# kensho-technologies/pyctcdecode

Hardware: NVIDIA H100
Metric: logit frames/sec decoded (batch, beam=100) (higher is better)
Workload: dtype f64

## Files before the change

include/b200ctc.h:

```cpp
#ifndef B200CTC_H
#define B200CTC_H

#include <stddef.h>
#include <stdint.h>

#ifdef __cplusplus
extern "C" {
#endif

#define B2C_E_OK 0
#define B2C_E_ARG (-1)
#define B2C_E_CUDA (-2)
#define B2C_E_IO (-3)
#define B2C_E_NOMEM (-4)
#define B2C_E_INTERNAL (-5)

#define B2C_DTYPE_F32 0
#define B2C_DTYPE_F64 1
#define B2C_DTYPE_F16 2
#define B2C_DTYPE_BF16 3

typedef struct b2c_lm b2c_lm_t;
typedef struct b2c_decoder b2c_decoder_t;
typedef struct b2c_result b2c_result_t;
// ... 98 lines not shown
    const int32_t* n_stream_toks;
    const uint32_t* stream_toks;
    int64_t n_stream_toks_total;
    const char* stream_pieces;
    size_t stream_pieces_size;
    const int32_t* stream_boundary;
} b2c_packed_t;
int b2c_result_packed(b2c_result_t* res, b2c_packed_t* out);
#define B2C_KIND_CONT 0
#define B2C_KIND_SPACE 1
#define B2C_KIND_BPE 2
int b2c_result_stream_beam(const b2c_result_t* res, int utt, int beam, int32_t aux[4], const uint32_t** toks, int* n_toks);
int b2c_result_n_frames(const b2c_result_t* res, int utt, int beam);
int b2c_hash_utf8(const char* s, uint64_t* hash, uint32_t* n_chars);
int b2c_hash_utf8_batch(const char* data, size_t size, int64_t count, uint64_t* hashes, uint32_t* n_chars);
int b2c_decoder_token_id(const b2c_decoder_t* dec, const char* label);

typedef struct {
    float ms_prepare;
    float ms_beam;
    float ms_total;
    int launches;
    long long h2d_bytes, d2h_bytes;
    long long frames;
    long long tokens;
    int cap_candidates;
    int cta_threads;
    int cta_slots;
    long long oversize_frames;
    int kernel_variant;
    long long cand_hist[7];
    long long inplace_frames;
    long long sorted_frames;
    int hinted;
} b2c_timings_t;
int b2c_decoder_last_timings(const b2c_decoder_t* dec, b2c_timings_t* out);
int b2c_decoder_last_tokens(const b2c_decoder_t* dec, int64_t* n_frames, int64_t* n_entries, int32_t* counts, uint32_t* ids,
                            double* lps, uint16_t* rec_id0, double* rec_lp0, int32_t* is_prob);

#ifdef __cplusplus
}
#endif
#endif
```

pyctcdecode_b200/_lib.py:

```python
import ctypes as C
import os
import threading

_HERE = os.path.dirname(os.path.abspath(__file__))
DEFAULT_LIBRARY = os.path.join(_HERE, "libb200ctc.so")

_lock = threading.Lock()
_lib = None
_lib_path = None


class LMState(C.Structure):
    _fields_ = [("words", C.c_uint32 * 5), ("backoff", C.c_float * 5), ("length", C.c_uint32)]


class StreamBeam(C.Structure):
    _fields_ = [("part_hash", C.c_uint64), ("logit_score", C.c_double), ("word_off", C.c_uint32), ("n_words", C.c_uint32),
                ("part_len", C.c_uint32), ("last_tok", C.c_uint32), ("pf_s", C.c_int32), ("pf_e", C.c_int32)]


class StreamState(C.Structure):
    _fields_ = [("beams", C.POINTER(StreamBeam)), ("n_beams", C.c_int), ("processed_frames", C.c_int),
                ("word_hashes", C.POINTER(C.c_uint64)), ("word_lens", C.POINTER(C.c_uint32)), ("n_words", C.c_int)]

# ... 15 lines not shown
        ("stream_states", C.POINTER(StreamState)),
        ("finalize_mode", C.c_int),
        ("text_only", C.c_int),
    ]


class Packed(C.Structure):
    _fields_ = [("n_utts", C.c_int32), ("n_models", C.c_int32), ("n_beams_total", C.c_int64), ("n_words_total", C.c_int64),
                ("n_beams", C.POINTER(C.c_int32)), ("scores", C.POINTER(C.c_double)), ("n_words", C.POINTER(C.c_int32)),
                ("frames", C.POINTER(C.c_int32)), ("texts", C.c_void_p), ("texts_size", C.c_size_t),
                ("states", C.POINTER(LMState)), ("stream_aux", C.POINTER(C.c_int32)), ("n_stream_toks", C.POINTER(C.c_int32)),
                ("stream_toks", C.POINTER(C.c_uint32)), ("n_stream_toks_total", C.c_int64),
                ("stream_pieces", C.c_void_p), ("stream_pieces_size", C.c_size_t), ("stream_boundary", C.POINTER(C.c_int32))]


class Timings(C.Structure):
    _fields_ = [
        ("ms_prepare", C.c_float),
        ("ms_beam", C.c_float),
        ("ms_total", C.c_float),
        ("launches", C.c_int),
        ("h2d_bytes", C.c_longlong),
        ("d2h_bytes", C.c_longlong),
        ("frames", C.c_longlong),
        ("tokens", C.c_longlong),
        ("cap_candidates", C.c_int),
        ("cta_threads", C.c_int),
        ("cta_slots", C.c_int),
        ("oversize_frames", C.c_longlong),
        ("kernel_variant", C.c_int),
        ("cand_hist", C.c_longlong * 7),
        ("inplace_frames", C.c_longlong),
        ("sorted_frames", C.c_longlong),
        ("hinted", C.c_int),
    ]


def _declare(L):
    vp, cp, i32, f64 = C.c_void_p, C.c_char_p, C.c_int, C.c_double
    pp = C.POINTER(vp)
    L.b2c_last_error.restype = cp
    L.b2c_version.restype = i32
    L.b2c_device_count.restype = i32
    L.b2c_lm_build_from_arpa.argtypes = [cp, C.POINTER(cp), C.c_long, pp]
    L.b2c_lm_build_from_file.argtypes = [cp, C.POINTER(cp), C.c_long, pp]
    L.b2c_lm_blob.argtypes = [vp, pp, C.POINTER(C.c_size_t)]
    L.b2c_lm_from_blob.argtypes = [vp, C.c_size_t, pp]
    L.b2c_lm_upload.argtypes = [vp, i32]
    L.b2c_lm_adopt_device_blob.argtypes = [vp, i32, vp, C.c_size_t]
    L.b2c_lm_destroy.argtypes = [vp]
    L.b2c_lm_destroy.restype = None
    L.b2c_lm_order.argtypes = [vp]
    L.b2c_lm_contains.argtypes = [vp, cp]
    L.b2c_lm_in_unigrams.argtypes = [vp, cp]
    L.b2c_lm_has_prefix.argtypes = [vp, cp]
    L.b2c_lm_have_unigrams.argtypes = [vp]
    L.b2c_lm_begin_sentence.argtypes = [vp, C.POINTER(LMState)]
    L.b2c_lm_begin_sentence.restype = None
    L.b2c_lm_null_context.argtypes = [vp, C.POINTER(LMState)]
    L.b2c_lm_null_context.restype = None
    L.b2c_lm_base_score.argtypes = [vp, C.POINTER(LMState), cp, C.POINTER(LMState)]
    L.b2c_lm_base_score.restype = C.c_float
    L.b2c_decoder_create.argtypes = [C.POINTER(cp), i32, i32, vp, i32, pp]
    L.b2c_decoder_destroy.argtypes = [vp]
    L.b2c_decoder_destroy.restype = None
    L.b2c_decoder_set_params.argtypes = [vp, f64, f64, f64, i32]
# ... 85 lines not shown
```

pyctcdecode_b200/csrc/b2c_api.cu:

```cuda
#include <algorithm>
#include <chrono>
#include <cmath>
#include <cstdint>
#include <cstdlib>
#include <cstring>
#include <map>
#include <memory>
#include <mutex>
#include <numeric>
#include <string>
#include <thread>
#include <atomic>
#include <condition_variable>
#include <functional>
#include <vector>

#ifdef B2C_HOSTSIM
#include "cuda_shim.h"
#else
#include <cuda_runtime.h>
#endif

#include "../../include/b200ctc.h"
#include "b2c_beam.h"
// ... 607 lines not shown
    for (size_t i = 0; i < br.words.size(); ++i) {
        if (i) br.text += ' ';
        br.text += br.words[i];
    }
    br.frames.resize(static_cast<size_t>(nw) * 2);
    for (int w = 0; w < nw; ++w) {
        br.frames[2 * w] = frames[2 * (nw - 1 - w)];
        br.frames[2 * w + 1] = frames[2 * (nw - 1 - w) + 1];
    }
    const size_t n = std::min(br.words.size(), static_cast<size_t>(nw));
    br.words.resize(n);
    br.frames.resize(n * 2);
}

static const int kNumCaps = 6;
static const u32 kCaps[kNumCaps] = {128, 256, 512, 1024, 2048, 4096};
static int threads_of(int c) { return kCaps[c] <= 128 ? 32 : (kCaps[c] <= 256 ? 64 : (kCaps[c] >= 2048 ? 256 : 128)); }
static int per_sm_of(u32 smem_bytes, int threads) {
    const int by_smem = static_cast<int>(std::max<u64>(1, (224 * 1024) / std::max<u32>(smem_bytes + 1024, 2048)));
    return std::min(by_smem, threads == 32 ? 8 : (threads == 64 ? 4 : (threads >= 256 ? 1 : 2)));
}

struct Launch { int cls; size_t ord_off; int count; B2cLayout L; int slots; int per_sm; int threads; int v5; };
struct Geometry {
    int n_utts = 0, V = 0, beam_width = 0, W_tab = 0, n_lm = 1, s_max_beams = 0, T_max = 0;
    u64 s_max_words = 0, total_frames = 0;
    size_t esz = 4;
    bool streaming = false, hint_ok = false, pipelined = false;
    u32 smem_budget = 0;
    const int32_t* T = nullptr;
    const int* order = nullptr;
};
struct Knobs {
    bool host_prof, no_pipe, no_hinted, force_v5, no_v5, no_lean, force_lean, pipe_all, no_gate, gate_early;
    int v5_variant, force_chunks;
};
static bool env_set(const char* name) { return std::getenv(name) != nullptr; }
static Knobs read_knobs() {
    Knobs k;
    k.host_prof = env_set("B200CTC_HOST_PROFILE");
    k.no_pipe = env_set("B200CTC_NO_PIPELINE") || !env_switch("B200CTC_PIPELINE", B2C_DEFAULT_PIPELINE != 0);
    k.no_hinted = env_set("B200CTC_NO_HINTED");
    k.force_v5 = env_set("B200CTC_FORCE_V5");
    k.no_v5 = env_set("B200CTC_NO_V5");
    const char* v = std::getenv("B200CTC_V5_VARIANT"), *fc = std::getenv("B200CTC_FORCE_CHUNKS");
    k.v5_variant = v ? std::max(0, std::min(2, std::atoi(v))) : -1;
    k.no_lean = env_set("B200CTC_NO_LEAN") || !env_switch("B200CTC_LEAN", B2C_DEFAULT_LEAN != 0);
    k.force_lean = env_set("B200CTC_FORCE_LEAN");
    k.force_chunks = fc ? std::atoi(fc) : 0;
    k.pipe_all = env_set("B200CTC_PIPELINE_ALL"); k.no_gate = env_set("B200CTC_NO_GATE");
    k.gate_early = env_set("B200CTC_HOSTSIM_GATE_EARLY");
    return k;
}
struct Plan {
    std::vector<Launch> launches;
    std::vector<int> ord;
    bool use_v5 = false, use_lean = false;
    int v5_variant = 0;
    std::vector<int> bounds;
    bool gated = false;
    bool redo_plain = false;
};

struct MetaLayout {
    size_t T, run, ord, next, ptr, bytes;
    explicit MetaLayout(int n = 0)
        : T(al16(8ull * n)), run(T + al16(4ull * n)), ord(run + al16(8ull * (n + 1))), next(ord + 2 * al16(4ull * n)), ptr(next + 64),
          bytes(ptr + al16(8ull * n)) {}
};
struct OutViews {
    int *nbeams, *status; double* scores; int *ntok, *nwords; B2cLmState* states;
    int* aux;
    B2cLmState* states_x;
};
struct OutLayout {
    u64 st = 0, sc = 0, nt = 0, nw = 0, ls = 0, ax = 0, lx = 0, bytes = 0;
    bool has_aux = false, has_x = false;
    OutLayout() = default;
    OutLayout(int n, int OB, int n_lm, bool streaming)
        : st(al16(4ull * n)), sc(st + al16(4ull * n)), nt(sc + al16(16ull * OB * n)), nw(nt + al16(4ull * OB * n)), ls(nw + al16(4ull * OB * n)),
          ax(ls + al16(sizeof(B2cLmState) * static_cast<u64>(OB) * n)), lx(ax + (streaming ? al16(16ull * OB * n) : 0)),
          bytes(lx + al16(sizeof(B2cLmState) * static_cast<u64>(OB) * n * static_cast<u64>(n_lm - 1))), has_aux(streaming), has_x(n_lm > 1) {}
    OutViews at(u8* b) const {
        return OutViews{reinterpret_cast<int*>(b), reinterpret_cast<int*>(b + st), reinterpret_cast<double*>(b + sc),
// ... 633 lines not shown
            const b2c_stream_state_t& ss = o->stream_states[i];
            if (ss.n_beams < 0 || ss.n_beams > 65535 || (ss.n_beams > 0 && !ss.beams)) return fail(B2C_E_ARG, "bad stream state");
            const B2cStreamUtt su{static_cast<u32>(c.s_beams.size()), static_cast<u32>(ss.n_beams), ss.processed_frames, 0};
            const u32 wbase = static_cast<u32>(c.s_wh.size());
            u64 words = 0;
            for (int b = 0; b < ss.n_beams; ++b) {
                const b2c_stream_beam_t& ib = ss.beams[b];
                if (static_cast<u64>(ib.word_off) + ib.n_words > static_cast<u64>(std::max(ss.n_words, 0)))
                    return fail(B2C_E_ARG, "stream beam word range outside the state's word list");
                if (ib.last_tok != B2C_NO_TOK && ib.last_tok >= static_cast<u32>(g.V)) return fail(B2C_E_ARG, "stream beam last_tok out of range");
                const u32 last = ib.last_tok == B2C_NO_TOK ? B2C_NO_TOK : d->toks[ib.last_tok].canon;
                c.s_beams.push_back(B2cStreamBeam{ib.part_hash, ib.logit_score, wbase + ib.word_off, ib.n_words, ib.part_len, last, ib.pf_s, ib.pf_e});
                words += ib.n_words;
            }
            for (int w = 0; w < ss.n_words; ++w) { c.s_wh.push_back(ss.word_hashes[w]); c.s_wl.push_back(ss.word_lens[w]); }
            c.s_utts[i] = su;
            g.s_max_beams = std::max(g.s_max_beams, ss.n_beams);
            g.s_max_words = std::max(g.s_max_words, words);
        }
    }
    g.W_tab = std::max(o->beam_width, g.s_max_beams);
    return 0;
}

static int make_params(b2c_decoder* d, Call& c) {
    const b2c_decode_opts_t* o = c.opts;
    B2cParams& P = c.P;
    P.V = c.g.V; P.is_bpe = d->is_bpe; P.has_dup_labels = d->has_dup_labels;
    P.beam_width = o->beam_width; P.prune_history = o->prune_history ? 1 : 0; P.out_beams = c.OB; P.narrow_chain = c.text_only ? 1 : 0;
    P.prune_logp = o->beam_prune_logp; P.token_min_logp = o->token_min_logp;
    P.alpha = d->alpha; P.beta = d->beta; P.unk_offset = d->unk;
    P.log_base_change = 0x1.26bb1bbb55516p+1;
    P.score_boundary = d->score_boundary; P.hot_weight = o->hotword_weight; P.bucket_scale = b2c_bucket_scale(o->beam_prune_logp);
    P.toks = d->d_toks.as<B2cTok>();
    if (d->lm) {
        auto it = d->lm->dev.find(d->device);
        if (it == d->lm->dev.end()) return fail(B2C_E_INTERNAL, "language model is not resident on this device");
        P.lm = d->lm->host.view(it->second);
        if (P.lm.order > B2C_MAX_ORDER) return fail(B2C_E_ARG, "n-gram order too large");
        P.n_lm = 1 + static_cast<int>(d->lmx.size());
    }
    int max_order = P.lm.order;
    std::vector<B2cLmExtra> lmx_host(d->lmx.size());
    for (size_t j = 0; j < d->lmx.size(); ++j) {
        const b2c_decoder::ExtraLm& x = d->lmx[j];
        auto it = x.lm->dev.find(d->device);
        if (it == x.lm->dev.end()) return fail(B2C_E_INTERNAL, "language model is not resident on this device");
        B2cLmExtra& X = lmx_host[j];
        std::memset(&X, 0, sizeof(X));
        X.lm = x.lm->host.view(it->second);
        if (X.lm.order > B2C_MAX_ORDER) return fail(B2C_E_ARG, "n-gram order too large");
        X.alpha = x.alpha; X.beta = x.beta; X.unk_offset = x.unk; X.score_boundary = x.score_boundary;
        max_order = std::max(max_order, X.lm.order);
    }
    if (!lmx_host.empty()) {
        if (d->d_lmx.ensure(sizeof(B2cLmExtra) * lmx_host.size())) return B2C_E_NOMEM;
        CUDA_OK(cudaMemcpy(d->d_lmx.p, lmx_host.data(), sizeof(B2cLmExtra) * lmx_host.size(), cudaMemcpyHostToDevice));
        P.lmx = d->d_lmx.as<B2cLmExtra>();
    }
    c.g.n_lm = std::max(1, P.n_lm);
    P.hist_n = std::max(1, max_order - 1);
    build_hot(o, c.hot, P.n_hot, P.hot_min_len_all);
    if (d->d_hot.ensure(c.hot.size() * sizeof(B2cHot))) return B2C_E_NOMEM;
    P.hot = d->d_hot.as<B2cHot>(); P.hot_mask = c.hot.size() - 1;
    return 0;
}
// ... 315 lines not shown
    return 0;
}

static int read_outputs(b2c_decoder* d, const Call& c, bool frames) {
    CUDA_OK(cudaMemcpyAsync(d->h_out_small.p, d->d_out_small.p, c.out.bytes, cudaMemcpyDeviceToHost, d->stream));
    CUDA_OK(cudaMemcpyAsync(d->h_out_toks.p, d->d_out_toks.p, c.tok_bytes, cudaMemcpyDeviceToHost, d->stream));
    if (frames) CUDA_OK(cudaMemcpyAsync(d->h_out_frames.p, d->d_out_frames.p, c.frm_bytes, cudaMemcpyDeviceToHost, d->stream));
    return 0;
}

static int read_back(b2c_decoder* d, Call& c) {
    const int n = c.g.n_utts;
    cudaStream_t st = d->stream;
    B2C_TRY(read_outputs(d, c, !c.text_only));
    if (d->h_mstats.ensure(64)) return B2C_E_NOMEM;
    CUDA_OK(cudaMemcpyAsync(d->h_mstats.p, d->d_mstats.p, 64, cudaMemcpyDeviceToHost, st));
    if (c.g.pipelined) CUDA_OK(cudaMemcpyAsync(d->h_sumk.p, d->d_sumk.p, 4ull * n, cudaMemcpyDeviceToHost, st));
    CUDA_OK(cudaEventRecord(d->ev[4], st));
    c.hp.mark(2);
    CUDA_OK(cudaStreamSynchronize(st));
    c.hp.mark(3);
    if (c.g.pipelined && d->h_maxk.as<u32>()[0] != 0) return B2C_E_RETRY_PLAIN;
    if (c.gated_call) {
        const int* status = c.out.at(d->h_out_small.as<u8>()).status;
        for (int i = 0; i < n; ++i) if (status[i] & B2C_ERR_GATE) { d->pipe_refused = true; return B2C_E_RETRY_PLAIN; }
    }
    d->tm.d2h_bytes += static_cast<long long>(c.out.bytes + c.tok_bytes + (c.text_only ? 0 : c.frm_bytes) + 8ull * n + 32);
    const u32* ms = d->h_mstats.as<u32>();
    d->hint_valid = true;
    d->hint_beam = c.opts->beam_width; d->hint_lm = c.P.lm.order > 0 ? 1 : 0; d->hint_hot = c.P.n_hot > 0 ? 1 : 0; d->hint_prune = c.P.prune_history;
    for (int q = 0; q < 6; ++q) d->hint_over[q] = ms[q];
    d->hint_frames = ms[6];
    for (int q = 0; q < 7; ++q) d->tm.cand_hist[q] = ms[q];
    d->tm.inplace_frames = ms[7]; d->tm.sorted_frames = ms[8];
    d->hint_wide_utts = ms[9]; d->hint_utts = ms[10];
    d->tm.oversize_frames = 0;
    for (int q = 0; q < 6; ++q)
        if (static_cast<int>(128u << q) == d->tm.cap_candidates) d->tm.oversize_frames = ms[q];
    return 0;
}

static int retry_failed(b2c_decoder* d, Call& c) {
    const int n = c.g.n_utts;
    cudaStream_t st = d->stream;
    const int* status = c.out.at(d->h_out_small.as<u8>()).status;
    std::vector<int> failed;
    for (int i = 0; i < n; ++i) if (status[i] != B2C_OK) failed.push_back(i);
    if (c.plan.use_lean && 10 * failed.size() > static_cast<size_t>(n)) d->lean_bad = true;
    for (int pass = 0; pass < 2 && !failed.empty(); ++pass) {
        bool only_slots = c.plan.use_lean && pass == 0;
        for (int i : failed) only_slots = only_slots && status[i] == B2C_ERR_SLOTS;
        if (pass == 0 && !only_slots) continue;
        int cls = kNumCaps;
        if (only_slots) {
            c.plan.use_lean = false;
            cls = 0;
            for (const Launch& l0 : c.plan.launches) if (l0.v5 >= 0) cls = l0.cls;
        }
        const Launch ln = plan_launch(c.g, c.maxk, c.plan, d->n_sm, failed, cls, !only_slots, static_cast<size_t>(n));
        if (ln.L.smem_bytes > d->smem_optin) return fail(B2C_E_ARG, "beam_width too large for the shared-memory selection arrays");
        if (d->d_ws.ensure(static_cast<u64>(ln.slots) * ln.L.gws_bytes)) return B2C_E_NOMEM;
        int* h_ord = c.h_ord();
        for (size_t i = 0; i < failed.size(); ++i) h_ord[n + i] = failed[i];
        CUDA_OK(cudaMemcpyAsync(c.d_ord() + n, h_ord + n, 4 * failed.size(), cudaMemcpyHostToDevice, st));
        CUDA_OK(cudaMemsetAsync(c.d_next() + 15, 0, 4, st));
        c.BA.L = ln.L; c.BA.n_utts = ln.count; c.BA.order = c.d_ord() + n; c.BA.next = c.d_next() + 15; c.BA.gws = d->d_ws.as<u8>();
        c.BA.chunk_t1 = 0;
        B2C_TRY(launch_beam(d, c.BA, ln, st, false));
        B2C_TRY(read_outputs(d, c, true));
        CUDA_OK(cudaStreamSynchronize(st));
        std::vector<int> still;
        for (int i : failed) if (status[i] != B2C_OK) still.push_back(i);
        failed.swap(still);
    }
    for (int i : failed)
        return fail(B2C_E_INTERNAL, "beam kernel workspace overflow (status " + std::to_string(status[i]) + ")");
    return 0;
}

static int record_timings(b2c_decoder* d, const Call& c) {
#if defined(B2C_PHASE_CLOCKS)
    {
        u64 hc[32];
        CUDA_OK(cudaMemcpy(hc, d->d_clk.p, sizeof(hc), cudaMemcpyDeviceToHost));
        std::fprintf(stderr, "[b2c phase clocks, summed over CTAs, Mcycles]");
        for (int q = 0; q < 24; ++q) std::fprintf(stderr, " p%d=%.3f", q, hc[q] / 1e6);
        std::fprintf(stderr, "  frames=%llu\n", static_cast<unsigned long long>(c.g.total_frames));
    }
#endif
    const int n_chunks = static_cast<int>(c.plan.bounds.size()) - 1;
    float ms = 0.f;
    if (c.chunk_timing) {
        float mp = 0.f, mb = 0.f;
        for (int ch = 0; ch < n_chunks; ++ch) {
            if (cudaEventElapsedTime(&ms, d->chunk_ev[3 * ch], d->chunk_ev[3 * ch + 1]) == cudaSuccess) mp += ms;
            if (!c.gated_call && cudaEventElapsedTime(&ms, d->chunk_ev[3 * ch + 1], d->chunk_ev[3 * ch + 2]) == cudaSuccess) mb += ms;
        }
        if (c.gated_call && cudaEventElapsedTime(&ms, d->ev[5], d->ev[3]) == cudaSuccess) mb = ms;
        d->tm.ms_prepare = mp; d->tm.ms_beam = mb;
        if (c.k.host_prof) {
            std::fprintf(stderr, "[b2c pipeline, ms after the call's first event]");
            for (int ch = 0; ch < n_chunks; ++ch) {
                float a0 = 0.f, a1 = 0.f, a2 = 0.f;
                cudaEventElapsedTime(&a0, d->ev[0], d->chunk_ev[3 * ch]);
                cudaEventElapsedTime(&a1, d->ev[0], d->chunk_ev[3 * ch + 1]);
                if (!c.gated_call) cudaEventElapsedTime(&a2, d->ev[0], d->chunk_ev[3 * ch + 2]);
                std::fprintf(stderr, "  chunk %d: copied %.3f streamed %.3f decoded %.3f", ch, a0, a1, a2);
            }
            float a4 = 0.f;
            cudaEventElapsedTime(&a4, d->ev[0], d->ev[4]);
            std::fprintf(stderr, "  d2h done %.3f\n", a4);
        }
    } else {
        if (!c.g.pipelined && cudaEventElapsedTime(&ms, d->ev[1], d->ev[2]) == cudaSuccess) d->tm.ms_prepare = ms;
        if (cudaEventElapsedTime(&ms, d->ev[5], d->ev[3]) == cudaSuccess) d->tm.ms_beam = ms;
    }
    if (cudaEventElapsedTime(&ms, d->ev[0], d->ev[4]) == cudaSuccess) d->tm.ms_total = ms;
    d->tm.frames = static_cast<long long>(c.g.total_frames);
    d->last_device_ms = static_cast<double>(d->tm.ms_prepare) + static_cast<double>(d->tm.ms_beam);
// ... 305 lines not shown
```

pyctcdecode_b200/csrc/b2c_beam.h:

```cpp
#pragma once
#include "b2c_cta.h"
#include "b2c_lm.h"

#if defined(__CUDACC__)
#define B2C_HDN __host__ __device__ __noinline__
#else
#define B2C_HDN __attribute__((noinline))
#endif

struct B2cBeamTab {
    double* logit;
    double* lm_hw;
    double* pscore;
    u64* text_hash;
    u64* part_hash;
    u64* hist_hash;
    u32* text_node;
    u32* chain;
    int* pf_s;
    int* pf_e;
    u16* last_tok;
    u16* part_len;
};

struct B2cScalars {
    u64 max_key;
    double prev_max;
    u32 n_beams, n_sel, n_new, chain_used, text_used, status, force_break;
    u32 flags;
    u32 m_over[6];
    u32 m_frames;
    u32 inplace_bad;
    u32 m_inplace;
    u32 clean_s, clean_g;
};
enum { B2C_FL_BPE = 1, B2C_FL_PRUNE = 2, B2C_FL_LM = 4, B2C_FL_PSCORE = 8 };

#define B2C_NBUCKET 256
#define B2C_NBUCKET_WIDE 2048
#define B2C_MAXWARPS 8
#define B2C_STAGE_K 64

struct B2cCandTier {
    u32 cap;
    u32 ht_cap;
    u64* ckey;
    double* cfold;
    u64* cth;
    u64* cph;
    u32* cmeta;
    u32* cslot;
    u32* cnext;
    u32* clast;
    u32* ht_idx;
    u32* ht_min;
    u32* ht_max;
    u32* ht_cnt;
};

struct B2cWork {
    B2cScalars* sc;
    B2cBeamTab cur, nxt;
    B2cCandTier tier_s, tier_g;
    u32* ord;
    u64* phk;
    u32* pslot;
    u32* pt_idx;
    u32* pt_min;
    u32 pt_cap;
// ... 882 lines not shown
}

struct B2cStreamIn {
    const B2cStreamBeam* beams;
    u32 n_beams;
    const u64* word_hash;
    const u32* word_len;
};
B2C_HDN void b2c_utt_begin(B2cParams P, B2cWork W, const B2cLmState* start_state, int K_first, B2cStreamIn in) {
    const u32 M0 = static_cast<u32>(K_first > 0 ? K_first : 1) * (in.n_beams > 0 ? in.n_beams : 1u);
    {
        const B2cCandTier C0 = b2c_pick_tier(W, M0);
        b2c_clear_tables(W, C0, b2c_ht_size(M0));
    }
    B2C_LEADER {
        B2cScalars* sc = W.sc;
        {
            const bool g0 = M0 > W.tier_s.cap && W.tier_g.cap > W.tier_s.cap;
            sc->clean_s = g0 ? 0u : b2c_ht_size(M0);
            sc->clean_g = g0 ? b2c_ht_size(M0) : 0u;
        }
        sc->n_beams = 1;
        sc->chain_used = 0;
        sc->text_used = 1;
        sc->status = B2C_OK;
        sc->force_break = 0;
        sc->inplace_bad = 0;
        sc->prev_max = 0.0;
        u32 fl = 0;
        if (P.is_bpe) fl |= B2C_FL_BPE;
        if (P.prune_history) fl |= B2C_FL_PRUNE;
        if (P.lm.order > 0) fl |= B2C_FL_LM;
        if (P.n_hot > 0 || P.lm.order > 0) fl |= B2C_FL_PSCORE;
        sc->flags = fl;
        B2cText root;
        for (int w = 0; w < B2C_MAX_HIST; ++w) { root.win[w] = 0; root.st.words[w] = 0; root.st.backoff[w] = 0.0f; }
        root.n_win = 0;
        root.hist_hash = B2C_HIST_SEED;
        root.raw_lm = 0.0;
        root.hw_count = 0;
        root.st.length = 0;
        if (P.lm.order > 0) {
            if (start_state) {
                root.st = *start_state;
            } else if (P.score_boundary) {
                root.st.length = 1;
                root.st.words[0] = P.lm.bos_id;
                root.st.backoff[0] = P.lm.uni[P.lm.bos_id].backoff;
            }
        }
        W.text[0] = root;
        if (P.n_lm > 1) {
            B2cLmState* x = b2c_text_states_x(W.text, W.text_cap, P.n_lm, 0);
            for (int j = 1; j < P.n_lm; ++j) {
                B2cLmState st;
                st.length = 0;
                for (int w = 0; w < B2C_MAX_HIST; ++w) { st.words[w] = 0; st.backoff[w] = 0.0f; }
                if (start_state) {
                    st = start_state[j];
                } else if (P.lmx[j - 1].score_boundary) {
                    st.length = 1;
                    st.words[0] = P.lmx[j - 1].lm.bos_id;
                    st.backoff[0] = P.lmx[j - 1].lm.uni[P.lmx[j - 1].lm.bos_id].backoff;
                }
                x[j - 1] = st;
            }
// ... 197 lines not shown
```

pyctcdecode_b200/csrc/b2c_beam_fast.h:

```cpp
#pragma once
#include <cstddef>
#include "b2c_beam.h"

#define B2C_FAST_KS 32
#define B2C_FAST_HR 32
#define B2C_FAST_TR 8
#define B2C_FAST_RMAX 6
#define B2C_FAST_NW 4

#if defined(__CUDA_ARCH__)
#define B2C_LAST_THREAD if (threadIdx.x == blockDim.x - 1)
#define B2C_IN_LAST_WARP if ((threadIdx.x >> 5) == (blockDim.x >> 5) - 1)
#define B2C_FOR_LANES(i, n) for (int i = static_cast<int>(threadIdx.x & 31); i < static_cast<int>(n); i += 32)
#else
#define B2C_LAST_THREAD if (true)
#define B2C_IN_LAST_WARP if (true)
#define B2C_FOR_LANES(i, n) B2C_FOR(i, n)
#endif

constexpr u32 b2c_pt_cap_c(int W) {
    u32 p = 16;
    while (p < 2u * static_cast<u32>(W)) p <<= 1;
    return p;
}
// ... 902 lines not shown
        nx.logit[r] = cur.logit[b] + slp[k];
        nx.lm_hw[r] = cur.lm_hw[b];
        nx.pscore[r] = same ? cur.pscore[b] : 0.0;
        nx.text_hash[r] = cur.text_hash[b];
        nx.part_hash[r] = nph;
        nx.hist_hash[r] = hh;
        nx.text_node[r] = cur.text_node[b];
        nx.chain[r] = chain;
        nx.pf_s[r] = pfs;
        nx.pf_e[r] = pfe;
        nx.last_tok[r] = ti.canon;
        nx.part_len[r] = static_cast<u16>(nplen);
        if (prune) {
            const u64 hk = b2c_fast_key(hh, nph, nplen & 0xFFFFu, ti.canon);
            S.phk[r] = hk;
            b2c_fence_block();
            u32 slot = static_cast<u32>(hk) & ptmask;
            while (true) {
                const u32 rep = b2c_atomic_cas_u32(&S.pt_idx[slot], B2C_NONE_U32, static_cast<u32>(r));
                if (rep == B2C_NONE_U32) break;
                b2c_fence_block();
                if (S.phk[rep] == hk) break;
                slot = (slot + 1) & ptmask;
            }
            S.pslot[r] = slot;
            b2c_atomic_min_u32(&S.pt_min[slot], static_cast<u32>(r));
        }
    }
    B2C_FOR(w, B2C_FAST_NW) { S.wmax[w] = w == 0 ? b2c_f64_key(top) : 0ull; }
    B2C_LAST_THREAD { S.holes = prune ? 1u : 0u; }
    return true;
}

template <int WC, int CAP, int LT>
B2C_HDN void b2c_fast_compact(B2cFastSmem<WC, CAP, LT>* Sp, int par) {
    B2cFastSmem<WC, CAP, LT>& S = *Sp;
    const B2cFastTab<WC>& cur = S.tab[par];
    B2cFastTab<WC>& nx = S.tab[par ^ 1];
    const u32 n = b2c_max_slots(S.wtop);
    const bool holes = S.holes != 0;
    const double prev_max = b2c_key_f64(b2c_max_slots(S.wmax));
    B2C_FOR(b, n) { S.ord[b] = (!holes || S.pt_min[S.pslot[b]] == static_cast<u32>(b)) ? 1u : 0u; }
    B2C_SYNC();
    B2C_FOR(b, n) {
        if (!S.ord[b]) continue;
        u32 j = 0;
        for (int q = 0; q < b; ++q) j += S.ord[q];
        nx.logit[j] = cur.logit[b]; nx.lm_hw[j] = cur.lm_hw[b]; nx.pscore[j] = cur.pscore[b];
        nx.text_hash[j] = cur.text_hash[b]; nx.part_hash[j] = cur.part_hash[b]; nx.hist_hash[j] = cur.hist_hash[b];
        nx.text_node[j] = cur.text_node[b]; nx.chain[j] = cur.chain[b];
        nx.pf_s[j] = cur.pf_s[b]; nx.pf_e[j] = cur.pf_e[b];
        nx.last_tok[j] = cur.last_tok[b]; nx.part_len[j] = cur.part_len[b];
    }
    B2C_SYNC();
    if (holes) {
        B2C_FOR(r, n) {
            const u32 s = S.pslot[r];
            S.pt_idx[s] = B2C_NONE_U32;
            S.pt_min[s] = B2C_NONE_U32;
        }
    }
    B2C_LEADER {
        u32 live = 0;
        for (u32 q = 0; q < n; ++q) live += S.ord[q];
        S.sc.n_beams = live;
        S.sc.n_sel = 0;
// ... 215 lines not shown
                if (has_ptk) ptk = A.P.toks[S.rid[(t + 1) & TM][threadIdx.x]];
            }
#endif
            B2C_FMARK(16);
            bool in_place = false;
            int done_frames = 0;
            if (oversize) {
                const u64 base_a = (f0 + static_cast<u64>(t & ~(B2C_RUN - 1))) * static_cast<u64>(V) + h.off;
                const int K_next = t + 1 < te ? static_cast<int>(S.rh[(t + 1) & HM].cnt) : 1;
                b2c_fast_compact<WC, CAP, LT>(&S, par);
                par ^= 1;
                b2c_fast_slow_step<WC, CAP, LT>(A.P, L, smem, g, par, t, A.tok_ids + base_a, A.tok_lp + base_a, K, K_next);
                done_frames = 1;
            } else {
                B2C_LAST_THREAD {
                    for (int c = 0; c < 6; ++c) st_over[c] += (Mq > (128u << c)) ? 1u : 0u;
                }
                if (kind == B2C_CHEAP_T3P) {
                    in_place = b2c_fast_scored_step<WC, CAP, LT>(A.P, S, chain_arena, par, t, sb, slot);
                    done_frames = in_place ? 1 : 0;
                } else if (kind != B2C_CHEAP_NO) {
                    done_frames = b2c_fast_run_step<WC, CAP, LT>(A.P, S, chain_arena, par, t, sb, R);
                    in_place = done_frames > 0;
                }
                if (in_place) {
                    B2C_LAST_THREAD { st_inplace += static_cast<u32>(done_frames); }
                    B2C_FMARK(5);
                } else if (kind == B2C_CHEAP_NO && b2c_fast_sorted_ok<WC, CAP, LT>(A.P, S, sb, slot, K, prev_single)) {
                    if (b2c_fast_sorted_step<WC, CAP, LT>(A.P, S, chain_arena, par, t, sb, slot, K, prev_single)) {
                        done_frames = 1;
                        B2C_LAST_THREAD { ++st_sorted; }
                        B2C_FMARK(7);
                    }
                }
                if (done_frames == 0) {
#if defined(B2C_PHASE_CLOCKS) && defined(__CUDA_ARCH__)
                    const long long c0 = clock64();
#endif
                    b2c_fast_step<WC, CAP, LT>(A.P, S, chain_arena, text_arena, text_cap, par, t, sb, slot, K);
#if defined(B2C_PHASE_CLOCKS) && defined(__CUDA_ARCH__)
                    if (threadIdx.x == 0) {
                        const int cls = K == 1 ? 0 : (K == 2 ? 1 : 2);
                        S.pclk[9 + cls] += static_cast<u64>(clock64() - c0);
                        S.pclk[12 + cls] += 1;
                    }
#endif
                    done_frames = 1;
                }
                B2C_LAST_THREAD { st_frames += static_cast<u32>(done_frames); }
            }
            const int t_last = t + done_frames - 1;
            if (done_frames == 1) prev_single = (K == 1) ? static_cast<u32>(b2c_fast_tok0<WC, CAP, LT>(A.P, S, t, sb).canon) : B2C_NONE_U32;
            else prev_single = static_cast<u32>(S.ltab[S.rh[t_last & HM].id0].canon);
            const int tn = t + done_frames;
#if defined(__CUDA_ARCH__)
            if (LT == 0) {
                if (has_ptk) S.stok[sb ^ 1][threadIdx.x] = ptk;
            }
#else
            if (LT == 0 && tn < te) {
                const u32 cn = S.rh[tn & HM].cnt;
                const u32 kb = cn < static_cast<u32>(KR) ? cn : static_cast<u32>(KR);
                B2C_FOR(c, kb) { S.stok[sb ^ 1][c] = A.P.toks[S.rid[tn & TM][c]]; }
            }
#endif
            B2C_FMARK(19);
            b2c_cp_async_wait_all();
            B2C_SYNC();
            B2C_FMARK(6);
            if (!in_place) par ^= 1;
            sb ^= 1;
            t = tn;
            if (gated && t >= te && te < Tn) {
                B2C_LEADER {
#if defined(__CUDA_ARCH__)
                    const volatile u32* flag = A.gate + gate_c + 1;
                    const long long c0 = clock64();
// ... 95 lines not shown
```

pyctcdecode_b200/csrc/b2c_common.h:

```cpp
#pragma once
#include <stdint.h>

#if defined(__CUDACC__)
#define B2C_HD __host__ __device__ __forceinline__
#define B2C_D __device__ __forceinline__
#else
#define B2C_HD inline
#define B2C_D inline
#endif

typedef unsigned long long u64;
typedef unsigned int u32;
typedef unsigned short u16;
typedef unsigned char u8;

#define B2C_MAX_ORDER 6
#define B2C_MAX_HIST (B2C_MAX_ORDER - 1)
#define B2C_NONE_U32 0xFFFFFFFFu
#define B2C_NO_TOK 0xFFFFu

#define B2C_P61 0x1FFFFFFFFFFFFFFFull
#define B2C_HASH_BASE 0x0A3B1C5D7E9F2461ull

B2C_HD u64 b2c_mod61(u64 lo, u64 hi) {
// ... 95 lines not shown
};

struct B2cHot { u64 key; u32 min_len; u32 is_word; };

#define B2C_MAX_LMS 4
struct B2cLmExtra {
    B2cLmView lm;
    double alpha, beta, unk_offset;
    int score_boundary;
    int pad;
};

struct B2cParams {
    int V;
    int is_bpe;
    int has_dup_labels;
    int beam_width;
    int prune_history;
    int hist_n;
    int out_beams;
    int narrow_chain;
    double prune_logp;
    double token_min_logp;
    double alpha, beta, unk_offset, log_base_change;
    int score_boundary;
    int n_hot;
    int hot_min_len_all;
    double hot_weight;
    double bucket_scale;
    const B2cHot* hot; u64 hot_mask;
    const B2cTok* toks;
    B2cLmView lm;
    int n_lm;
    int pad_lm;
    const B2cLmExtra* lmx;
};

enum { B2C_CK_CONT = 0, B2C_CK_SPACE = 1, B2C_CK_BPE = 2, B2C_CK_ROOT = 3 };
struct B2cChain {
    u32 parent;
    u16 tok;
    u8 kind;
    u8 has_word;
    int ws, we;
};
B2C_HD void b2c_chain_store(B2cChain* arena, u32 id, const B2cChain& c, bool narrow) {
    if (narrow) {
        reinterpret_cast<u64*>(arena)[id] = static_cast<u64>(c.parent) | (static_cast<u64>(c.tok) << 32) |
                                            (static_cast<u64>(c.kind) << 48) | (static_cast<u64>(c.has_word) << 56);
    } else {
        arena[id] = c;
    }
}
B2C_HD B2cChain b2c_chain_load(const B2cChain* arena, u32 id, bool narrow) {
    if (!narrow) return arena[id];
    const u64 v = reinterpret_cast<const u64*>(arena)[id];
    B2cChain c;
    c.parent = static_cast<u32>(v);
    c.tok = static_cast<u16>(v >> 32);
    c.kind = static_cast<u8>(v >> 48);
    c.has_word = static_cast<u8>(v >> 56);
    c.ws = -1;
    c.we = -1;
    return c;
}
struct B2cText {
    u64 win[B2C_MAX_HIST];
// ... 29 lines not shown
```

Measured before the change: 49.60 million.

## Add single-token fast path for frames with one surviving candidate token

Adds a specialized beam step for frames where only one non-space token survives the token threshold and no LM/hotword scoring or BPE is active. It extends every beam with that token, detects merges and pruning via a shared hash table and a block-wide vote, and updates beams in place when nothing merges or gets pruned. Otherwise it falls back to a bucketed rank-and-write path or to the general step. This avoids the full candidate generation and sort for such frames, but adds complexity and can waste the speculative pass when it has to fall back. The path can be disabled with an environment variable.

```diff
diff --git a/include/b200ctc.h b/include/b200ctc.h
--- a/include/b200ctc.h
+++ b/include/b200ctc.h
@@ -154,6 +154,7 @@
     long long cand_hist[7];
     long long inplace_frames;
     long long sorted_frames;
+    long long single_frames;
     int hinted;
 } b2c_timings_t;
 int b2c_decoder_last_timings(const b2c_decoder_t* dec, b2c_timings_t* out);
diff --git a/pyctcdecode_b200/_lib.py b/pyctcdecode_b200/_lib.py
--- a/pyctcdecode_b200/_lib.py
+++ b/pyctcdecode_b200/_lib.py
@@ -71,6 +71,7 @@
         ("cand_hist", C.c_longlong * 7),
         ("inplace_frames", C.c_longlong),
         ("sorted_frames", C.c_longlong),
+        ("single_frames", C.c_longlong),
         ("hinted", C.c_int),
     ]
 
diff --git a/pyctcdecode_b200/csrc/b2c_api.cu b/pyctcdecode_b200/csrc/b2c_api.cu
--- a/pyctcdecode_b200/csrc/b2c_api.cu
+++ b/pyctcdecode_b200/csrc/b2c_api.cu
@@ -663,7 +663,7 @@
     const int* order = nullptr;
 };
 struct Knobs {
-    bool host_prof, no_pipe, no_hinted, force_v5, no_v5, no_lean, force_lean, pipe_all, no_gate, gate_early;
+    bool host_prof, no_pipe, no_hinted, force_v5, no_v5, no_lean, force_lean, pipe_all, no_gate, gate_early, no_single;
     int v5_variant, force_chunks;
 };
 static bool env_set(const char* name) { return std::getenv(name) != nullptr; }
@@ -681,6 +681,7 @@
     k.force_chunks = fc ? std::atoi(fc) : 0;
     k.pipe_all = env_set("B200CTC_PIPELINE_ALL"); k.no_gate = env_set("B200CTC_NO_GATE");
     k.gate_early = env_set("B200CTC_HOSTSIM_GATE_EARLY");
+    k.no_single = env_set("B200CTC_NO_SINGLE_STEP");
     return k;
 }
 struct Plan {
@@ -1380,6 +1381,7 @@
     P.alpha = d->alpha; P.beta = d->beta; P.unk_offset = d->unk;
     P.log_base_change = 0x1.26bb1bbb55516p+1;
     P.score_boundary = d->score_boundary; P.hot_weight = o->hotword_weight; P.bucket_scale = b2c_bucket_scale(o->beam_prune_logp);
+    P.kflags = c.k.no_single ? B2C_FL_NO_SINGLE : 0;
     P.toks = d->d_toks.as<B2cTok>();
     if (d->lm) {
         auto it = d->lm->dev.find(d->device);
@@ -1761,7 +1763,7 @@
     for (int q = 0; q < 6; ++q) d->hint_over[q] = ms[q];
     d->hint_frames = ms[6];
     for (int q = 0; q < 7; ++q) d->tm.cand_hist[q] = ms[q];
-    d->tm.inplace_frames = ms[7]; d->tm.sorted_frames = ms[8];
+    d->tm.inplace_frames = ms[7]; d->tm.sorted_frames = ms[8]; d->tm.single_frames = ms[11];
     d->hint_wide_utts = ms[9]; d->hint_utts = ms[10];
     d->tm.oversize_frames = 0;
     for (int q = 0; q < 6; ++q)
@@ -1812,8 +1814,8 @@
     {
         u64 hc[32];
         CUDA_OK(cudaMemcpy(hc, d->d_clk.p, sizeof(hc), cudaMemcpyDeviceToHost));
-        std::fprintf(stderr, "[b2c phase clocks, summed over CTAs, Mcycles]");
-        for (int q = 0; q < 24; ++q) std::fprintf(stderr, " p%d=%.3f", q, hc[q] / 1e6);
+        std::fprintf(stderr, "[b2c phase clocks, summed over CTAs, cycles or frames]");
+        for (int q = 0; q < 32; ++q) std::fprintf(stderr, " p%d=%llu", q, static_cast<unsigned long long>(hc[q]));
         std::fprintf(stderr, "  frames=%llu\n", static_cast<unsigned long long>(c.g.total_frames));
     }
 #endif
diff --git a/pyctcdecode_b200/csrc/b2c_beam.h b/pyctcdecode_b200/csrc/b2c_beam.h
--- a/pyctcdecode_b200/csrc/b2c_beam.h
+++ b/pyctcdecode_b200/csrc/b2c_beam.h
@@ -34,7 +34,7 @@
     u32 m_inplace;
     u32 clean_s, clean_g;
 };
-enum { B2C_FL_BPE = 1, B2C_FL_PRUNE = 2, B2C_FL_LM = 4, B2C_FL_PSCORE = 8 };
+enum { B2C_FL_BPE = 1, B2C_FL_PRUNE = 2, B2C_FL_LM = 4, B2C_FL_PSCORE = 8, B2C_FL_NO_SINGLE = 16 };
 
 #define B2C_NBUCKET 256
 #define B2C_NBUCKET_WIDE 2048
@@ -983,6 +983,7 @@
         if (P.prune_history) fl |= B2C_FL_PRUNE;
         if (P.lm.order > 0) fl |= B2C_FL_LM;
         if (P.n_hot > 0 || P.lm.order > 0) fl |= B2C_FL_PSCORE;
+        fl |= static_cast<u32>(P.kflags) & B2C_FL_NO_SINGLE;
         sc->flags = fl;
         B2cText root;
         for (int w = 0; w < B2C_MAX_HIST; ++w) { root.win[w] = 0; root.st.words[w] = 0; root.st.backoff[w] = 0.0f; }
diff --git a/pyctcdecode_b200/csrc/b2c_beam_fast.h b/pyctcdecode_b200/csrc/b2c_beam_fast.h
--- a/pyctcdecode_b200/csrc/b2c_beam_fast.h
+++ b/pyctcdecode_b200/csrc/b2c_beam_fast.h
@@ -958,6 +958,306 @@
     return true;
 }
 
+template <int CAP, int LT>
+constexpr bool b2c_fast_has_single() { return CAP >= 1024 && LT > 0; }
+
+template <int WC, int CAP, int LT>
+B2C_HD bool b2c_fast_single_ok(const B2cFastSmem<WC, CAP, LT>& S, int sb, int slot, int K, u32 prev_single) {
+    if (!b2c_fast_has_single<CAP, LT>() || K != 1 || prev_single != B2C_NONE_U32) return false;
+    if (S.sc.flags & (B2C_FL_PSCORE | B2C_FL_BPE | B2C_FL_NO_SINGLE)) return false;
+    return (b2c_fast_tok<WC, CAP, LT>(S, sb, slot, 0).flags & B2C_TF_SPACE) == 0;
+}
+
+struct B2cSingleItem {
+    double lg;
+    u64 nph;
+    u32 slots;
+    u32 meta;
+};
+enum { B2C_SI_T3 = 1u << 16, B2C_SI_LIVE = 1u << 17, B2C_SI_LEAD = 1u << 18, B2C_SI_LAST = 19 };
+B2C_HD u32 b2c_sync_or(u32 v) {
+#if defined(__CUDA_ARCH__)
+    return static_cast<u32>(__syncthreads_or(static_cast<int>(v)));
+#else
+    return v;
+#endif
+}
+
+template <int WC, int CAP, int LT>
+B2C_HD int b2c_fast_single_step(const B2cParams& P, B2cFastSmem<WC, CAP, LT>& S, B2cChain* chain_arena, int par, int t, int sb,
+                                int slot) {
+    typedef B2cFastSmem<WC, CAP, LT> SM;
+    B2cFastTab<WC>& cur = S.tab[par];
+    B2cFastTab<WC>& nx = S.tab[par ^ 1];
+    const u32 n = b2c_max_slots(S.wtop);
+    const bool prune = (S.sc.flags & B2C_FL_PRUNE) != 0;
+    const bool holes = S.holes != 0;
+    const double ref = b2c_key_f64(b2c_max_slots(S.wmax));
+    constexpr u32 hmask = SM::HT - 1, ptmask = SM::PT - 1;
+    constexpr u32 PTAG = 0x80000000u;
+    const B2cTok& ti = b2c_fast_tok<WC, CAP, LT>(S, sb, slot, 0);
+    const u32 canon = ti.canon;
+    const bool blank = (ti.flags & B2C_TF_BLANK) != 0;
+    const double p = S.rlp[slot][0];
+    const bool t0 = blank || cur.last_tok[0] == canon;
+    const double top = b2c_combine_score(false, cur.logit[0] + p, cur.lm_hw[0], t0 ? cur.pscore[0] : 0.0, 0u);
+#if defined(__CUDA_ARCH__)
+    B2cSingleItem items[1];
+#define B2C_SITEM(b) items[0]
+#else
+    B2cSingleItem items[WC];
+#define B2C_SITEM(b) items[b]
+#endif
+
+    B2C_FOR(s, B2C_NBUCKET) { S.bcnt[s] = 0; S.bhead[s] = B2C_NONE_U32; }
+    u32 vote = 0;
+    B2C_FOR(b, n) {
+        B2cSingleItem& it = B2C_SITEM(b);
+        const u32 ub = static_cast<u32>(b);
+        it.meta = 0;
+        if (holes && S.pt_min[S.pslot[b]] != ub) continue;
+        const u64 ph = cur.part_hash[b];
+        const u32 plen = cur.part_len[b];
+        const bool t3 = !blank && cur.last_tok[b] != canon;
+        it.nph = t3 ? b2c_hash_append(ph, ti.raw_hash, ti.raw_pow) : ph;
+        const u32 nplen = t3 ? plen + ti.raw_nchars : plen;
+        it.lg = cur.logit[b] + p;
+        S.cfold[b] = it.lg;
+        const u64 key = b2c_fast_key(cur.text_hash[b], it.nph, nplen, canon);
+        S.ckey[b] = key;
+        u64 hk = 0;
+        if (prune) {
+            hk = b2c_fast_key(cur.hist_hash[b], it.nph, nplen & 0xFFFFu, canon);
+            S.phk[b] = hk;
+        }
+        b2c_fence_block();
+        u32 hs = static_cast<u32>(key) & hmask;
+        bool claimed = false;
+        while (true) {
+            const u32 rep = b2c_atomic_cas_u32(&S.ht_idx[hs], B2C_NONE_U32, ub);
+            if (rep == B2C_NONE_U32) { claimed = true; break; }
+            b2c_fence_block();
+            if (!(rep & PTAG) && S.ckey[rep] == key) break;
+            hs = (hs + 1) & hmask;
+        }
+        if (!claimed) {
+            b2c_atomic_min_u32(&S.ht_min[hs], ub);
+            b2c_atomic_max_u32(&S.ht_max[hs], ub);
+            if (b2c_atomic_add_u32(&S.ht_cnt[hs], 1u) >= 2u) b2c_atomic_or_u32(&S.cheap_bad, 1u);
+            vote = 1;
+        }
+        u32 psl = SM::HT;
+        if (prune) {
+            u32 q = static_cast<u32>(hk) & hmask;
+            while (true) {
+                const u32 rep = b2c_atomic_cas_u32(&S.ht_idx[q], B2C_NONE_U32, ub | PTAG);
+                if (rep == B2C_NONE_U32) { psl = q; break; }
+                b2c_fence_block();
+                if ((rep & PTAG) && S.phk[rep & ~PTAG] == hk) { vote = 1; break; }
+                q = (q + 1) & hmask;
+            }
+        }
+        it.slots = hs | (psl << 16);
+        it.meta = (nplen & 0xFFFFu) | (t3 ? B2C_SI_T3 : 0u) | B2C_SI_LIVE;
+        const double sco = b2c_combine_score(false, it.lg, cur.lm_hw[b], t3 ? 0.0 : cur.pscore[b], nplen);
+        if (!(sco >= top + P.prune_logp)) vote = 1;
+    }
+    vote = b2c_sync_or(vote);
+
+    if (!vote) {
+        B2C_FOR(b, n) {
+            const B2cSingleItem& it = B2C_SITEM(b);
+            if (!(it.meta & B2C_SI_LIVE)) {
+                cur.logit[b] = cur.logit[b] + p;
+                continue;
+            }
+            S.ht_idx[it.slots & 0xFFFFu] = B2C_NONE_U32;
+            S.ht_idx[it.slots >> 16] = B2C_NONE_U32;
+            const int ps0 = cur.pf_s[b], pe0 = cur.pf_e[b];
+            cur.logit[b] = it.lg;
+            cur.last_tok[b] = static_cast<u16>(canon);
+            if (!(it.meta & B2C_SI_T3)) {
+                if (!blank) cur.pf_e[b] = t + 1;
+            } else {
+                const u32 id = static_cast<u32>(t) * static_cast<u32>(WC) + static_cast<u32>(b);
+                B2cChain c;
+                c.parent = cur.chain[b];
+                c.tok = static_cast<u16>(S.rid[slot][0]);
+                c.kind = B2C_CK_CONT;
+                c.has_word = 0;
+                c.ws = ps0;
+                c.we = pe0;
+                b2c_chain_store(chain_arena, id, c, P.narrow_chain != 0);
+                cur.chain[b] = id;
+                cur.part_hash[b] = it.nph;
+                cur.part_len[b] = static_cast<u16>(it.meta);
+                cur.pscore[b] = 0.0;
+                cur.pf_s[b] = ps0 < 0 ? t : ps0;
+                cur.pf_e[b] = t + 1;
+            }
+        }
+        B2C_FOR(w, B2C_FAST_NW) { S.wmax[w] = w == 0 ? b2c_f64_key(top) : 0ull; }
+        B2C_FMARK(24);
+        return 2;
+    }
+    if (S.cheap_bad) {
+        B2C_FOR(b, n) {
+            const B2cSingleItem& it = B2C_SITEM(b);
+            if (!(it.meta & B2C_SI_LIVE)) continue;
+            const u32 hs = it.slots & 0xFFFFu;
+            S.ht_idx[hs] = B2C_NONE_U32;
+            S.ht_min[hs] = B2C_NONE_U32;
+            S.ht_max[hs] = 0;
+            S.ht_cnt[hs] = 0;
+            S.ht_idx[it.slots >> 16] = B2C_NONE_U32;
+        }
+        B2C_SYNC();
+        B2C_LEADER { S.cheap_bad = 0; }
+        return 0;
+    }
+
+    if (holes) {
+        B2C_FOR(r, n) {
+            const u32 s = S.pslot[r];
+            S.pt_idx[s] = B2C_NONE_U32;
+            S.pt_min[s] = B2C_NONE_U32;
+        }
+    }
+    {
+        u64 tmax = 0;
+        B2C_FOR(b, n) {
+            B2cSingleItem& it = B2C_SITEM(b);
+            if (!(it.meta & B2C_SI_LIVE)) continue;
+            const u32 ub = static_cast<u32>(b);
+            const u32 hs = it.slots & 0xFFFFu;
+            const u32 c0 = S.ht_idx[hs];
+            const u32 cnt = S.ht_cnt[hs] + 1;
+            u32 first = c0, last = c0, mid = c0;
+            if (cnt > 1) {
+                const u32 lo = S.ht_min[hs], hi = S.ht_max[hs];
+                first = lo < c0 ? lo : c0;
+                last = hi > c0 ? hi : c0;
+                mid = c0 + lo + hi - first - last;
+            }
+            if (first != ub) continue;
+            double s = it.lg;
+            if (cnt == 3) s = b2c_sum_log_scores_ool(s, S.cfold[mid]);
+            if (cnt > 1) s = b2c_sum_log_scores_ool(s, S.cfold[last]);
+            it.lg = s;
+            u32 meta = it.meta;
+            if (last != ub) {
+                const u64 ph = cur.part_hash[last];
+                const u32 plen = cur.part_len[last];
+                const bool t3 = !blank && cur.last_tok[last] != canon;
+                it.nph = t3 ? b2c_hash_append(ph, ti.raw_hash, ti.raw_pow) : ph;
+                meta = ((t3 ? plen + ti.raw_nchars : plen) & 0xFFFFu) | (t3 ? B2C_SI_T3 : 0u) | B2C_SI_LIVE;
+            }
+            it.meta = meta | B2C_SI_LEAD | (last << B2C_SI_LAST);
+            const u32 nplen = meta & 0xFFFFu;
+            const double sco = b2c_combine_score(false, s, cur.lm_hw[last], (meta & B2C_SI_T3) ? 0.0 : cur.pscore[last], nplen);
+            const u64 key = b2c_f64_key(sco);
+            S.ckey[b] = key;
+            const u32 bkt = b2c_bucket(ref, sco, P.bucket_scale);
+            b2c_atomic_add_u32(&S.bcnt[bkt], 1u);
+#if defined(__CUDA_ARCH__)
+            S.cnext[b] = atomicExch(&S.bhead[bkt], ub);
+#else
+            S.cnext[b] = S.bhead[bkt];
+            S.bhead[bkt] = ub;
+#endif
+            if (key > tmax) tmax = key;
+        }
+        b2c_warp_max_u64_slot(tmax, S.wmax);
+    }
+    B2C_SYNC();
+
+    u32* const bpre = S.bpre[b2c_warp_id()];
+    b2c_bucket_scan_warp_v(S.bcnt, bpre);
+    const double thr = b2c_key_f64(b2c_max_slots(S.wmax)) + P.prune_logp;
+    const u32 width = static_cast<u32>(P.beam_width);
+    {
+        u32 my_top = 0;
+        B2C_FOR(b, n) {
+            const B2cSingleItem& it = B2C_SITEM(b);
+            if (!(it.meta & B2C_SI_LIVE)) continue;
+            {
+                const u32 hs = it.slots & 0xFFFFu;
+                S.ht_idx[hs] = B2C_NONE_U32;
+                S.ht_min[hs] = B2C_NONE_U32;
+                S.ht_max[hs] = 0;
+                S.ht_cnt[hs] = 0;
+                S.ht_idx[it.slots >> 16] = B2C_NONE_U32;
+            }
+            if (!(it.meta & B2C_SI_LEAD)) continue;
+            const u64 key = S.ckey[b];
+            const double sco = b2c_key_f64(key);
+            if (!(sco >= thr)) continue;
+            const u32 bkt = b2c_bucket(ref, sco, P.bucket_scale);
+            u32 rank = bpre[bkt];
+            if (rank >= width) continue;
+            for (u32 j = S.bhead[bkt]; j != B2C_NONE_U32;) {
+                const u64 kj = S.ckey[j];
+                const u32 jn = S.cnext[j];
+                const u32 gt = kj > key ? 1u : 0u, eq_before = (kj == key ? 1u : 0u) & (j < static_cast<u32>(b) ? 1u : 0u);
+                rank += gt | eq_before;
+                j = jn;
+            }
+            if (rank >= width) continue;
+            if (rank + 1 > my_top) my_top = rank + 1;
+            const u32 bl = it.meta >> B2C_SI_LAST;
+            const u32 nplen = it.meta & 0xFFFFu;
+            const bool t3 = (it.meta & B2C_SI_T3) != 0;
+            const u64 hh = cur.hist_hash[bl];
+            if (prune) {
+                const u64 hk = b2c_fast_key(hh, it.nph, nplen, canon);
+                S.phk[rank] = hk;
+                b2c_fence_block();
+                u32 q = static_cast<u32>(hk) & ptmask;
+                while (true) {
+                    const u32 rep = b2c_atomic_cas_u32(&S.pt_idx[q], B2C_NONE_U32, rank);
+                    if (rep == B2C_NONE_U32) break;
+                    b2c_fence_block();
+                    if (S.phk[rep] == hk) break;
+                    q = (q + 1) & ptmask;
+                }
+                S.pslot[rank] = q;
+                b2c_atomic_min_u32(&S.pt_min[q], rank);
+            }
+            const int ps0 = cur.pf_s[bl], pe0 = cur.pf_e[bl];
+            u32 chain = cur.chain[bl];
+            if (t3) {
+                const u32 id = static_cast<u32>(t) * static_cast<u32>(WC) + rank;
+                B2cChain c;
+                c.parent = chain;
+                c.tok = static_cast<u16>(S.rid[slot][0]);
+                c.kind = B2C_CK_CONT;
+                c.has_word = 0;
+                c.ws = ps0;
+                c.we = pe0;
+                b2c_chain_store(chain_arena, id, c, P.narrow_chain != 0);
+                chain = id;
+            }
+            nx.logit[rank] = it.lg;
+            nx.text_hash[rank] = cur.text_hash[bl];
+            nx.part_hash[rank] = it.nph;
+            nx.part_len[rank] = static_cast<u16>(nplen);
+            nx.last_tok[rank] = static_cast<u16>(canon);
+            nx.pf_s[rank] = !t3 ? ps0 : (ps0 < 0 ? t : ps0);
+            nx.pf_e[rank] = (!t3 && blank) ? pe0 : t + 1;
+            nx.chain[rank] = chain;
+            nx.text_node[rank] = cur.text_node[bl];
+            nx.lm_hw[rank] = cur.lm_hw[bl];
+            nx.hist_hash[rank] = hh;
+            nx.pscore[rank] = t3 ? 0.0 : cur.pscore[bl];
+        }
+        b2c_warp_max_u32_slot(my_top, S.wtop);
+    }
+#undef B2C_SITEM
+    B2C_LAST_THREAD { S.holes = prune ? 1u : 0u; }
+    B2C_FMARK(24);
+    return 1;
+}
+
 template <int WC, int CAP, int LT>
 B2C_HDN void b2c_fast_compact(B2cFastSmem<WC, CAP, LT>* Sp, int par) {
     B2cFastSmem<WC, CAP, LT>& S = *Sp;
@@ -1239,6 +1539,17 @@
                         B2C_LAST_THREAD { ++st_sorted; }
                         B2C_FMARK(7);
                     }
+                } else if (b2c_fast_has_single<CAP, LT>() && kind == B2C_CHEAP_NO &&
+                           b2c_fast_single_ok<WC, CAP, LT>(S, sb, slot, K, prev_single)) {
+                    const int r = b2c_fast_single_step<WC, CAP, LT>(A.P, S, chain_arena, par, t, sb, slot);
+                    if (r > 0) {
+                        done_frames = 1;
+                        in_place = r == 2;
+                        if (A.m_stats) { B2C_LAST_THREAD { b2c_atomic_add_u32(A.m_stats + 11, 1u); } }
+                    }
+#if defined(B2C_PHASE_CLOCKS) && defined(__CUDA_ARCH__)
+                    if (threadIdx.x == 0) S.pclk[r == 0 ? 27 : (r == 2 ? 26 : 25)] += 1;
+#endif
                 }
                 if (done_frames == 0) {
 #if defined(B2C_PHASE_CLOCKS) && defined(__CUDA_ARCH__)
@@ -1247,9 +1558,9 @@
                     b2c_fast_step<WC, CAP, LT>(A.P, S, chain_arena, text_arena, text_cap, par, t, sb, slot, K);
 #if defined(B2C_PHASE_CLOCKS) && defined(__CUDA_ARCH__)
                     if (threadIdx.x == 0) {
-                        const int cls = K == 1 ? 0 : (K == 2 ? 1 : 2);
-                        S.pclk[9 + cls] += static_cast<u64>(clock64() - c0);
-                        S.pclk[12 + cls] += 1;
+                        const u64 dc = static_cast<u64>(clock64() - c0);
+                        if (K == 1 && prev_single != B2C_NONE_U32) { S.pclk[15] += dc; S.pclk[23] += 1; }
+                        else { const int cls = K == 1 ? 0 : (K == 2 ? 1 : 2); S.pclk[9 + cls] += dc; S.pclk[12 + cls] += 1; }
                     }
 #endif
                     done_frames = 1;
diff --git a/pyctcdecode_b200/csrc/b2c_common.h b/pyctcdecode_b200/csrc/b2c_common.h
--- a/pyctcdecode_b200/csrc/b2c_common.h
+++ b/pyctcdecode_b200/csrc/b2c_common.h
@@ -151,7 +151,7 @@
     const B2cTok* toks;
     B2cLmView lm;
     int n_lm;
-    int pad_lm;
+    int kflags;
     const B2cLmExtra* lmx;
 };
 
```

New measurement: 56.42 million (median of 6 runs). 13.8% higher.
